# jizongFox/MI-based-Regularized-Semi-supervised-Segmentation

Measured on NVIDIA B200. Metric: iic_mi_loss_fwd_bwd_mpixels_per_s, higher is better.
Workload: dtype f32

## Files before the change

mi-based-regularized-semi-supervised-segmentation_b200/csrc/local_bwd_tcrb10h.cu:

```cuda
#include <cuda_fp16.h>
#include <stdlib.h>

#include "common.cuh"
#include "local_kernels.cuh"
#include "tc_common.cuh"
#include "tma.cuh"

namespace iic {
namespace bwdrb10h {
using namespace tc;

constexpr int T = 3, PAD = 1;
constexpr int KP = 16;
constexpr int RMAX = 8;
constexpr int TBUF = 2 * RMAX * KP;
constexpr int APX = 272;
constexpr int MAXW = 248;
constexpr int A_CHUNK = APX * 16;
constexpr int A_SLOT = 4 * A_CHUNK;
constexpr int NA = 6;
constexpr int RAW_SLOT = 10 * 256 * 4;
constexpr int NRAW = 6;
constexpr int WROWS = T * KP;
constexpr int W_TILE = 2 * WROWS * 16;
constexpr int W_IMG = 6 * W_TILE;
constexpr int NTHREADS = 704;
constexpr int NTHREADS_FL = 704;
constexpr int SMEM_BYTES = NA * A_SLOT + 2 * W_IMG + NRAW * RAW_SLOT + 1024;
constexpr int NL = 4;
constexpr int SMEM_BYTES_FL = SMEM_BYTES + NL * RAW_SLOT;
constexpr float A_SCALE = 256.f;
constexpr int A_SCALE_LOG2 = 8;
constexpr int W_TARGET_LOG2 = 12;



#ifdef IIC_TC_TRACE
__device__ long long g_trace[4][64][6];
__device__ long long g_ctrace[32][8];
#define TRACE(role, slot) do { if (blockIdx.x == 0 && tt >= 16 && tt < 80) g_trace[role][tt - 16][slot] = clock64(); } while (0)
#define CTRACE(slot) do { if (blockIdx.x == 0 && i < 32) g_ctrace[i][slot] = clock64(); } while (0)
#else
#define TRACE(role, slot) do { } while (0)
#define CTRACE(slot) do { } while (0)
#endif

struct Params {
  int B, H, W, K;
  const float* Wc[2];
  int Kp4;
  const float* grad_loss;
  float* out[2];
  long long out_sn[2];
  int from_logits;
  float inv_temp;
  const float* lout[2];
  long long l_sn[2], l_sc[2], l_sh[2];
};

__device__ __forceinline__ uint32_t pack_h2(float a, float b) {
  const __half2 p = __floats2half2_rn(a, b);
  return *reinterpret_cast<const uint32_t*>(&p);
}
__device__ __forceinline__ uint4 pack_h8(const float* v) {
  return make_uint4(pack_h2(v[0], v[1]), pack_h2(v[2], v[3]), pack_h2(v[4], v[5]), pack_h2(v[6], v[7]));
}
__device__ __forceinline__ void split_h(float v, float& h, float& l) {
  h = __half2float(__float2half_rn(v));
  l = __half2float(__float2half_rn(v - h));
}

__device__ __forceinline__ void build_weight_row(const float* __restrict__ Wc, unsigned char* img, int e, int K, int Kp4, float wscale) {
  const int row = e % WROWS, tx = e / WROWS;
  const int ty = T - 1 - row / KP, o = row % KP;
  float w1[10], w2[10];
#pragma unroll
  for (int c = 0; c < 10; ++c) {
    const float v = (c < K && o < K) ? __ldg(Wc + ((size_t)c * T * T + ty * T + tx) * Kp4 + o) * wscale : 0.f;
    split_h(v, w1[c], w2[c]);
  }
  const float c0[8] = {w1[0], w1[1], w1[2], w1[3], w1[4], w1[5], w1[6], w1[7]};
  const float c1[8] = {w1[8], w1[9], w1[0], w1[1], w1[2], w1[3], w1[4], w1[5]};
  const float c2[8] = {w1[6], w1[7], w1[8], w1[9], w2[0], w2[1], w2[2], w2[3]};
  const float c3[8] = {w2[4], w2[5], w2[6], w2[7], w2[8], w2[9], 0.f, 0.f};
  uint4* t = reinterpret_cast<uint4*>(img + (size_t)tx * 2 * W_TILE);
  t[row] = pack_h8(c0);
  t[WROWS + row] = pack_h8(c1);
  t[2 * WROWS + row] = pack_h8(c2);
  t[3 * WROWS + row] = pack_h8(c3);
}

struct Chunk { int n, h0, nr, q0; bool cont_next; };
__device__ __forceinline__ Chunk next_chunk(long long r, long long R0, long long R1, int H, int rc) {
  Chunk c;
  c.n = (int)(r / H);
  c.h0 = (int)(r - (long long)c.n * H);
  int run = H - c.h0;
  if (run > R1 - r) run = (int)(R1 - r);
  c.nr = rc < run ? rc : run;
  if (run - c.nr == 1 && c.nr >= 3) c.nr -= 1;
  c.q0 = (r > R0 && c.h0 > 0) ? 2 : 0;
  c.cont_next = c.nr < run;
  return c;
}

template <bool FROM_LOGITS>
__global__ void __launch_bounds__(FROM_LOGITS ? NTHREADS_FL : NTHREADS, 1)
local_bwd_tcrb10h_kernel(const __grid_constant__ CUtensorMap map0, const __grid_constant__ CUtensorMap map1, const Params P) {
  extern __shared__ __align__(1024) unsigned char smem_dyn[];
  __shared__ __align__(8) uint64_t raw_full[NRAW], raw_empty[NRAW], a_full[NA], a_empty[NA], w_full, accum_full[2], tmem_ready[2];
  __shared__ __align__(8) uint64_t l_full[NL], l_empty[NL];
  __shared__ uint32_t tmem_base_s;
  __shared__ float wmax_s[4];
  __shared__ float unscale_s;
  unsigned char* smem = smem_dyn + ((1024u - (smem_u32(smem_dyn) & 1023u)) & 1023u);
  unsigned char* a_ring = smem;
  unsigned char* w_img = smem + NA * A_SLOT;
  unsigned char* raw_ring = w_img + 2 * W_IMG;
  unsigned char* l_ring = raw_ring + NRAW * RAW_SLOT;
  const int wid = threadIdx.x >> 5, lane = threadIdx.x & 31;
  const long long rows_total = (long long)P.B * P.H;
  const long long R0 = (long long)blockIdx.x * rows_total / gridDim.x;
  const long long R1 = (long long)(blockIdx.x + 1) * rows_total / gridDim.x;
  const int share = (int)(R1 - R0);
  const int nch = (share + RMAX - 1) / RMAX;
  const int rc = nch > 0 ? (share + nch - 1) / nch : RMAX;
  const int SW = P.W + 8;
  const int raw_bytes = P.K * SW * 4;
  const int ntile = P.W > 128 ? 2 : 1;

  if (threadIdx.x == 0) {
    for (int s = 0; s < NRAW; ++s) { mbar_init(&raw_full[s], 1); mbar_init(&raw_empty[s], 4); }
    for (int s = 0; s < NA; ++s) { mbar_init(&a_full[s], 4); mbar_init(&a_empty[s], 2); }
    mbar_init(&w_full, 4);
    const int ndset_i = ntile == 2 ? 2 : 1;
    for (int s = 0; s < 2; ++s) { mbar_init(&accum_full[s], 4); mbar_init(&tmem_ready[s], 4 * ndset_i); }
    for (int s = 0; s < NL; ++s) { mbar_init(&l_full[s], 1); mbar_init(&l_empty[s], 4 * ndset_i); }
    mbar_fence_init();
  }
  if (wid == 3) {
    asm volatile("tcgen05.alloc.cta_group::1.sync.aligned.shared::cta.b32 [%0], %1;" ::"r"(smem_u32(&tmem_base_s)), "r"(512));
    asm volatile("tcgen05.relinquish_alloc_permit.cta_group::1.sync.aligned;");
  }
  asm volatile("tcgen05.fence::before_thread_sync;");
  __syncthreads();
  asm volatile("tcgen05.fence::after_thread_sync;");
  const uint32_t tmem_base = tmem_base_s;

  if (wid == 0) {
    if (lane == 0) {
      tma_prefetch_desc(&map0);
      tma_prefetch_desc(&map1);
      int t = 0, s = 0;
      unsigned sph = 0;
      for (int sweep = 0; sweep < 2; ++sweep)
      for (long long r = R0; r < R1;) {
        const Chunk c = next_chunk(r, R0, R1, P.H, rc);
        for (int q = c.q0; q < c.nr + T - 1; ++q, ++t) {
          { const int tt = t; (void)tt; TRACE(0, 0); }
          if (t >= NRAW) mbar_wait(&raw_empty[s], sph ^ 1u, 1);
          { const int tt = t; (void)tt; TRACE(0, 1); }
          mbar_arrive_expect_tx(&raw_full[s], raw_bytes);
          tma_load_4d(raw_ring + s * RAW_SLOT, sweep == 0 ? &map0 : &map1, &raw_full[s], -4, c.h0 - PAD + q, 0, c.n);
          if (++s == NRAW) { s = 0; sph ^= 1u; }
        }
        r += c.nr;
      }
    }
  } else if (wid == 3) {
    if (FROM_LOGITS && lane == 0) {
      int t = 0, s = 0;
      unsigned sph = 0;
      for (int sweep = 0; sweep < 2; ++sweep)
      for (long long r = R0; r < R1;) {
        const Chunk c = next_chunk(r, R0, R1, P.H, rc);
        for (int orow = 0; orow < c.nr; ++orow, ++t) {
          if (t >= NL) mbar_wait(&l_empty[s], sph ^ 1u, 9);
          mbar_arrive_expect_tx(&l_full[s], raw_bytes);
          tma_load_4d(l_ring + s * RAW_SLOT, sweep == 0 ? &map1 : &map0, &l_full[s], -4, c.h0 + orow, 0, c.n);
          if (++s == NL) { s = 0; sph ^= 1u; }
        }
        r += c.nr;
      }
    }
  } else if (wid == 1 || wid == 2 || wid == 12 || wid == 13) {
    const int mt = (wid == 1 || wid == 12) ? 0 : 1;
    const int par = wid >= 12 ? 1 : 0;
    const bool mine = mt < ntile;
    mbar_wait(&w_full, 0u, 7);
    const uint64_t w_base0 = make_desc_kmajor_noswz(smem_u32(w_img), WROWS * 16);
    static_assert(NA % 2 == 0 && NRAW % 2 == 0, "the stage-parity split needs even ring depths");
    int a = 0, i = 0, tt = 0;
    unsigned aph = 0;
    for (int sweep = 0; sweep < 2; ++sweep)
    for (long long r = R0; r < R1; ++i) {
      const uint64_t w_base = w_base0 + (uint64_t)(sweep * (W_IMG / 16));
      const Chunk c = next_chunk(r, R0, R1, P.H, rc);
      const int buf = i & 1;
      if (lane == 0 && wid == 1) CTRACE(0);
      mbar_wait(&tmem_ready[buf], (unsigned)(i >> 1) & 1u, 6);
      if (lane == 0 && wid == 1) CTRACE(1);
      asm volatile("tcgen05.fence::after_thread_sync;");
      const int nq = c.nr + T - 1;
      const int nr_next = c.cont_next ? next_chunk(r + c.nr, R0, R1, P.H, rc).nr : 0;
      for (int q = c.q0; q < nq; ++q, ++tt) {
        if ((tt & 1) != par) {
          if (++a == NA) { a = 0; aph ^= 1u; }
          continue;
        }
        if (lane == 0 && par == 0) TRACE(1 + mt, 0);
        mbar_wait(&a_full[a], aph, 5);
        asm volatile("tcgen05.fence::after_thread_sync;");
        if (lane == 0) {
          if (par == 0) TRACE(1 + mt, 1);
          if (mine) {
            const int ty_max = q < T - 1 ? q : T - 1;
            const int ty_min = q - c.nr + 1 > 0 ? q - c.nr + 1 : 0;
            const uint32_t nn = (uint32_t)((ty_max - ty_min + 1) * KP);
            const uint32_t idesc_f16 = (1u << 4) | ((nn >> 3) << 17) | (8u << 24);
            const uint32_t d_tmem = tmem_base + (uint32_t)(buf * TBUF + (mt * RMAX + (q - ty_max)) * KP);
            const uint64_t a_12 = make_desc_kmajor_noswz(smem_u32(a_ring + a * A_SLOT), A_CHUNK) + (uint64_t)(mt * 128 + 8 - PAD);
            const uint64_t a_34 = a_12 + (uint64_t)(2 * A_CHUNK / 16);
            const uint64_t b_base = w_base + (uint64_t)((T - 1 - ty_max) * KP);
#pragma unroll
            for (int tx = 0; tx < T; ++tx) {
              const uint64_t bt = b_base + (uint64_t)tx * (2 * W_TILE / 16);
              umma_bf16(d_tmem, a_12 + (uint64_t)tx, bt, idesc_f16);
              umma_bf16(d_tmem, a_34 + (uint64_t)tx, bt + (uint64_t)(W_TILE / 16), idesc_f16);
            }
          }
        }
        if (c.cont_next && q >= c.nr) {
          mbar_wait(&tmem_ready[buf ^ 1], (unsigned)((i + 1) >> 1) & 1u, 6);
          asm volatile("tcgen05.fence::after_thread_sync;");
          if (lane == 0 && mine) {
            const int q2 = q - c.nr;
            const int ty_max = q2;
            const int ty_min = q2 - nr_next + 1 > 0 ? q2 - nr_next + 1 : 0;
            const uint32_t nn = (uint32_t)((ty_max - ty_min + 1) * KP);
            const uint32_t idesc_f16 = (1u << 4) | ((nn >> 3) << 17) | (8u << 24);
            const uint32_t d_tmem = tmem_base + (uint32_t)((buf ^ 1) * TBUF + (mt * RMAX + (q2 - ty_max)) * KP);
            const uint64_t a_12 = make_desc_kmajor_noswz(smem_u32(a_ring + a * A_SLOT), A_CHUNK) + (uint64_t)(mt * 128 + 8 - PAD);
            const uint64_t a_34 = a_12 + (uint64_t)(2 * A_CHUNK / 16);
            const uint64_t b_base = w_base + (uint64_t)((T - 1 - ty_max) * KP);
#pragma unroll
            for (int tx = 0; tx < T; ++tx) {
              const uint64_t bt = b_base + (uint64_t)tx * (2 * W_TILE / 16);
              umma_bf16(d_tmem, a_12 + (uint64_t)tx, bt, idesc_f16);
              umma_bf16(d_tmem, a_34 + (uint64_t)tx, bt + (uint64_t)(W_TILE / 16), idesc_f16);
            }
          }
        }
        if (lane == 0) {
          if (par == 0) TRACE(1 + mt, 2);
          umma_commit(&a_empty[a]);
        }
        __syncwarp();
        if (++a == NA) { a = 0; aph ^= 1u; }
      }
      if (lane == 0) umma_commit(&accum_full[buf]);
      __syncwarp();
      r += c.nr;
    }
  } else if (wid >= 4 && wid < 12) {
    const int tid = (threadIdx.x - 128) & 127;
    const int grp = wid >= 8 ? 1 : 0;
    int a = 0, s = 0, t = 0;
    unsigned aph = 0, sph = 0;
    for (int sweep = 0; sweep < 2; ++sweep)
    for (long long r = R0; r < R1;) {
      const Chunk c = next_chunk(r, R0, R1, P.H, rc);
      for (int q = c.q0; q < c.nr + T - 1; ++q, ++t) {
        if ((t & 1) != grp) {
          if (++a == NA) { a = 0; aph ^= 1u; }
          if (++s == NRAW) { s = 0; sph ^= 1u; }
          continue;
        }
        const int tt = t;
        (void)tt;
        if (tid == 0 && wid == 4) TRACE(3, 0);
        if (t >= NA) mbar_wait(&a_empty[a], aph ^ 1u, 3);
        if (tid == 0 && wid == 4) TRACE(3, 1);
        mbar_wait(&raw_full[s], sph, 4);
        if (tid == 0 && wid == 4) TRACE(3, 2);
        unsigned char* am = a_ring + a * A_SLOT;
        const float* raw = reinterpret_cast<const float*>(raw_ring + s * RAW_SLOT);
        const int srow = c.h0 - PAD + q;
        const bool row_in = srow >= 0 && srow < P.H;
        float v[2][10];
#pragma unroll
        for (int u = 0; u < 2; ++u) {
          const int px = tid + u * 128;
#pragma unroll
          for (int ch = 0; ch < 10; ++ch) v[u][ch] = (ch < P.K && px < SW) ? raw[ch * SW + px] : 0.f;
        }
#pragma unroll
        for (int u = 0; u < 2; ++u) {
          const int px = tid + u * 128;
          if (FROM_LOGITS) {
            const int col = px - 4;
            if (row_in && col >= 0 && col < P.W) {
              float mx = v[u][0];
#pragma unroll
              for (int ch = 1; ch < 10; ++ch) if (ch < P.K) mx = fmaxf(mx, v[u][ch]);
              float sum = 0.f;
#pragma unroll
              for (int ch = 0; ch < 10; ++ch) {
                v[u][ch] = ch < P.K ? __expf((v[u][ch] - mx) * P.inv_temp) : 0.f;
                sum += v[u][ch];
              }
              const float inv = 1.f / sum;
#pragma unroll
              for (int ch = 0; ch < 10; ++ch) v[u][ch] *= inv;
            } else {
#pragma unroll
              for (int ch = 0; ch < 10; ++ch) v[u][ch] = 0.f;
            }
          }
        }
        float2 hi[10], lo[10];
#pragma unroll
        for (int ch = 0; ch < 10; ++ch) {
          const float2 sv = __fmul2_rn(make_float2(v[0][ch], v[1][ch]), make_float2(A_SCALE, A_SCALE));
          hi[ch] = make_float2(__uint_as_float(__float_as_uint(sv.x) & 0xFFFFE000u), __uint_as_float(__float_as_uint(sv.y) & 0xFFFFE000u));
          lo[ch] = __ffma2_rn(hi[ch], make_float2(-1.f, -1.f), sv);
        }
#pragma unroll
        for (int u = 0; u < 2; ++u) {
          const int px = tid + u * 128;
          uint32_t hp[5], lp[5];
#pragma unroll
          for (int c2 = 0; c2 < 5; ++c2) {
            const __half2 hh = u == 0 ? __floats2half2_rn(hi[2 * c2].x, hi[2 * c2 + 1].x) : __floats2half2_rn(hi[2 * c2].y, hi[2 * c2 + 1].y);
            const __half2 ll = u == 0 ? __floats2half2_rn(lo[2 * c2].x, lo[2 * c2 + 1].x) : __floats2half2_rn(lo[2 * c2].y, lo[2 * c2 + 1].y);
            hp[c2] = *reinterpret_cast<const uint32_t*>(&hh);
            lp[c2] = *reinterpret_cast<const uint32_t*>(&ll);
          }
          if (px < SW) {
            const int off = (px + 4) * 16;
            *reinterpret_cast<uint4*>(am + off) = make_uint4(hp[0], hp[1], hp[2], hp[3]);
            *reinterpret_cast<uint4*>(am + A_CHUNK + off) = make_uint4(hp[4], lp[0], lp[1], lp[2]);
            *reinterpret_cast<uint4*>(am + 2 * A_CHUNK + off) = make_uint4(lp[3], lp[4], hp[0], hp[1]);
            *reinterpret_cast<uint4*>(am + 3 * A_CHUNK + off) = make_uint4(hp[2], hp[3], hp[4], 0u);
          }
        }
        __syncwarp();
        if (lane == 0) mbar_arrive(&raw_empty[s]);
        asm volatile("fence.proxy.async.shared::cta;" ::: "memory");
        __syncwarp();
        if (lane == 0) mbar_arrive(&a_full[a]);
        if (tid == 0 && wid == 4) TRACE(3, 3);
        if (++a == NA) { a = 0; aph ^= 1u; }
        if (++s == NRAW) { s = 0; sph ^= 1u; }
      }
      r += c.nr;
    }
  } else if (wid >= 14) {
    const int q4 = wid & 3;
    const int dset = wid >= 18 ? 1 : 0;
    const int ndset = ntile == 2 ? 2 : 1;
    const int mt0 = ndset == 2 ? dset : 0, mt1 = ndset == 2 ? dset + 1 : ntile;
    const int zc0 = ndset == 2 ? dset * RMAX * KP : 0, zc1 = ndset == 2 ? (dset + 1) * RMAX * KP : TBUF;
    float unscale = 1.f;
    const float g0 = P.grad_loss ? __ldg(P.grad_loss) : 1.f;
    const size_t plane = (size_t)P.H * P.W;
    const uint32_t lane_base = tmem_base + ((uint32_t)(q4 * 32) << 16);
    auto zero_accumulators = [&](int buf) {
      for (int c = zc0; c < zc1; c += 8)
        asm volatile("tcgen05.st.sync.aligned.32x32b.x8.b32 [%0], {%1, %1, %1, %1, %1, %1, %1, %1};" ::"r"(lane_base + buf * TBUF + c), "r"(0u) : "memory");
      asm volatile("tcgen05.wait::st.sync.aligned;" ::: "memory");
      asm volatile("tcgen05.fence::before_thread_sync;");
      __syncwarp();
      if (lane == 0) mbar_arrive(&tmem_ready[buf]);
    };
    if (dset < ndset) {
    zero_accumulators(0);
    zero_accumulators(1);
    }
    if (dset == 0) {
      const int etid = threadIdx.x - 14 * 32;
      const int ncoef = P.K * T * T * P.Kp4;
      float mx = 0.f;
      for (int e = etid; e < 2 * ncoef; e += 128) mx = fmaxf(mx, fabsf(__ldg(P.Wc[e >= ncoef] + (e >= ncoef ? e - ncoef : e))));
#pragma unroll
      for (int o = 16; o > 0; o >>= 1) mx = fmaxf(mx, __shfl_xor_sync(0xffffffffu, mx, o));
      if (lane == 0) wmax_s[q4] = mx;
      asm volatile("bar.sync 1, 128;" ::: "memory");
      mx = fmaxf(fmaxf(wmax_s[0], wmax_s[1]), fmaxf(wmax_s[2], wmax_s[3]));
      int wexp = 0;
      if (mx > 0.f && mx < 3.0e38f) wexp = W_TARGET_LOG2 - ilogbf(mx);
      if (wexp > 100) wexp = 100;
      const float wscale = scalbnf(1.f, wexp);
      unscale = scalbnf(1.f, -(wexp + A_SCALE_LOG2));
      for (int e = etid; e < 2 * 3 * WROWS; e += 128) {
        const int sweep = e / (3 * WROWS);
        build_weight_row(P.Wc[sweep], w_img + sweep * W_IMG, e - sweep * 3 * WROWS, P.K, P.Kp4, wscale);
      }
      if (etid == 0) unscale_s = unscale;
      asm volatile("fence.proxy.async.shared::cta;" ::: "memory");
      __syncwarp();
      if (lane == 0) mbar_arrive(&w_full);
    } else {
      mbar_wait(&w_full, 0u, 7);
      unscale = *reinterpret_cast<volatile float*>(&unscale_s);
    }
    const float g = g0 * unscale;
    int i = 0, ls = 0;
    unsigned lph = 0;
    for (int sweep = 0; sweep < 2 && dset < ndset; ++sweep)
    for (long long r = R0; r < R1; ++i) {
      const Chunk c = next_chunk(r, R0, R1, P.H, rc);
      const int buf = i & 1;
      if (lane == 0 && wid == 14) CTRACE(2);
      mbar_wait(&accum_full[buf], (unsigned)(i >> 1) & 1u, 8);
      if (lane == 0 && wid == 14) CTRACE(3);
      asm volatile("tcgen05.fence::after_thread_sync;");
      for (int orow = 0; orow < c.nr; orow += 2) {
        const int nrow = orow + 1 < c.nr ? 2 : 1;
        if (FROM_LOGITS) {
          mbar_wait(&l_full[ls], lph, 10);
          if (nrow == 2) mbar_wait(&l_full[(ls + 1) % NL], (ls + 1 == NL) ? (lph ^ 1u) : lph, 10);
        }
        for (int mt = mt0; mt < mt1; ++mt) {
          const int col = mt * 128 + q4 * 32 + lane;
          const bool live = col < P.W;
          uint32_t v[2][16];
#pragma unroll
          for (int h = 0; h < 2; ++h) {
            const int orh = orow + h < RMAX ? orow + h : orow;
#pragma unroll
            for (int ch = 0; ch < 16; ch += 8) {
              const uint32_t taddr = lane_base + (uint32_t)(buf * TBUF + (mt * RMAX + orh) * KP + ch);
              asm volatile("tcgen05.ld.sync.aligned.32x32b.x8.b32 {%0, %1, %2, %3, %4, %5, %6, %7}, [%8];"
                           : "=r"(v[h][ch]), "=r"(v[h][ch + 1]), "=r"(v[h][ch + 2]), "=r"(v[h][ch + 3]), "=r"(v[h][ch + 4]),
                             "=r"(v[h][ch + 5]), "=r"(v[h][ch + 6]), "=r"(v[h][ch + 7])
                           : "r"(taddr));
            }
          }
          asm volatile("tcgen05.wait::ld.sync.aligned;" ::: "memory");
          if (live) {
#pragma unroll
            for (int h = 0; h < 2; ++h) {
              if (h < nrow) {
                float* dst = P.out[sweep] + (size_t)c.n * P.out_sn[sweep] + (size_t)(c.h0 + orow + h) * P.W + col;
                if (!FROM_LOGITS) {
                  if (P.K == 10) {
#pragma unroll
                    for (int o = 0; o < 10; ++o) dst[(size_t)o * plane] = g * __uint_as_float(v[h][o]);
                  } else {
#pragma unroll
                    for (int o = 0; o < 9; ++o) dst[(size_t)o * plane] = g * __uint_as_float(v[h][o]);
                  }
                } else {
                  const float* lp = reinterpret_cast<const float*>(l_ring + ((ls + h) % NL) * RAW_SLOT) + col + 4;
                  float pr[10];
                  float mx = -3.0e38f;
#pragma unroll
                  for (int o = 0; o < 10; ++o) {
                    pr[o] = o < P.K ? lp[o * SW] : -3.0e38f;
                    mx = fmaxf(mx, pr[o]);
                  }
                  float sum = 0.f;
#pragma unroll
                  for (int o = 0; o < 10; ++o) {
                    pr[o] = o < P.K ? __expf((pr[o] - mx) * P.inv_temp) : 0.f;
                    sum += pr[o];
                  }
                  const float inv = 1.f / sum;
                  float dot = 0.f;
#pragma unroll
                  for (int o = 0; o < 10; ++o) {
                    pr[o] *= inv;
                    dot = fmaf(g * __uint_as_float(v[h][o]), pr[o], dot);
                  }
                  if (P.K == 10) {
#pragma unroll
                    for (int o = 0; o < 10; ++o) dst[(size_t)o * plane] = P.inv_temp * pr[o] * (g * __uint_as_float(v[h][o]) - dot);
                  } else {
#pragma unroll
                    for (int o = 0; o < 9; ++o) dst[(size_t)o * plane] = P.inv_temp * pr[o] * (g * __uint_as_float(v[h][o]) - dot);
                  }
                }
              }
            }
          }
        }
        if (FROM_LOGITS) {
          __syncwarp();
          for (int h = 0; h < nrow; ++h) {
            if (lane == 0) mbar_arrive(&l_empty[ls]);
            if (++ls == NL) { ls = 0; lph ^= 1u; }
          }
        }
      }
      r += c.nr;
      if (lane == 0 && wid == 14) CTRACE(4);
      zero_accumulators(buf);
      if (lane == 0 && wid == 14) CTRACE(5);
    }
  }
  asm volatile("tcgen05.fence::before_thread_sync;");
  __syncthreads();
  if (wid == 3) asm volatile("tcgen05.dealloc.cta_group::1.sync.aligned.b32 %0, %1;" ::"r"(tmem_base), "r"(512));
}

}

int local_bwd_tcrb10h_try(const LocalMaps& m, const float* Wx, const float* Wy, const LocalGrads& g, int from_logits,
                          float inv_temp, cudaStream_t st) {
  using namespace bwdrb10h;
  const int B = m.B, K = m.K, H = m.H, W = m.W, sms = m.sms;
  if ((K != 9 && K != 10) || m.pad != 1 || W % 4 != 0 || W > MAXW || W < 8) return -1;
  if ((long long)B * H < 8LL * sms && !options().tc10_force) return -1;
  CUtensorMap mx, my;
  if (!make_map_4d(&mx, m.x, m, W + 8, 1, K)) return -1;
  if (!make_map_4d(&my, m.y, m, W + 8, 1, K)) return -1;
  IIC_CHECK_RC(ensure_dyn_smem((const void*)(local_bwd_tcrb10h_kernel<false>), (int)(SMEM_BYTES)));
  IIC_CHECK_RC(ensure_dyn_smem((const void*)(local_bwd_tcrb10h_kernel<true>), (int)(SMEM_BYTES_FL)));
  const int Kp4 = (K + 3) & ~3;
  Params P{B, H, W, K, {Wx, Wy}, Kp4, g.grad_loss, {g.gx, g.gy}, {g.gx_sn, g.gy_sn}, from_logits, inv_temp, {m.x.p, m.y.p},
           {m.x.sn, m.y.sn}, {m.x.sc, m.y.sc}, {m.x.sh, m.y.sh}};
  if (from_logits) local_bwd_tcrb10h_kernel<true><<<sms, NTHREADS_FL, SMEM_BYTES_FL, st>>>(my, mx, P);
  else local_bwd_tcrb10h_kernel<false><<<sms, NTHREADS, SMEM_BYTES, st>>>(my, mx, P);
  IIC_CHECK_CUDA(cudaGetLastError());
  return 0;
}

}
```

Before: 9992.

## Fold horizontal taps into MMA N dimension and combine via warp shuffles

The backward local conv no longer issues three separate UMMA pairs per row, one per horizontal tap tx. It widens N to 32 so that all three tx taps for the 10 outputs come out of one MMA. The epilogue then shifts the tx=0 and tx=2 partial sums by one column with warp shuffles, using a small shared-memory exchange at warp boundaries, and adds them to the centre tap. Tiles overlap, at 126 columns per tile, to supply halo columns. RMAX is halved, the parity-split second MMA warp pair is removed, and chunk-boundary MMAs are deferred with held ring slots. The aim is fewer MMA issues and less weight footprint, at the cost of extra TMEM loads, shuffles and a named barrier in the epilogue.

```diff
diff --git a/mi-based-regularized-semi-supervised-segmentation_b200/csrc/local_bwd_tcrb10h.cu b/mi-based-regularized-semi-supervised-segmentation_b200/csrc/local_bwd_tcrb10h.cu
--- a/mi-based-regularized-semi-supervised-segmentation_b200/csrc/local_bwd_tcrb10h.cu
+++ b/mi-based-regularized-semi-supervised-segmentation_b200/csrc/local_bwd_tcrb10h.cu
@@ -11,9 +11,10 @@
 using namespace tc;
 
 constexpr int T = 3, PAD = 1;
-constexpr int KP = 16;
-constexpr int RMAX = 8;
-constexpr int TBUF = 2 * RMAX * KP;
+constexpr int TW = 126;
+constexpr int NO = 32;
+constexpr int RMAX = 4;
+constexpr int TBUF = 2 * RMAX * NO;
 constexpr int APX = 272;
 constexpr int MAXW = 248;
 constexpr int A_CHUNK = APX * 16;
@@ -21,11 +22,11 @@
 constexpr int NA = 6;
 constexpr int RAW_SLOT = 10 * 256 * 4;
 constexpr int NRAW = 6;
-constexpr int WROWS = T * KP;
+constexpr int WROWS = T * NO;
 constexpr int W_TILE = 2 * WROWS * 16;
-constexpr int W_IMG = 6 * W_TILE;
-constexpr int NTHREADS = 704;
-constexpr int NTHREADS_FL = 704;
+constexpr int W_IMG = 2 * W_TILE;
+constexpr int NTHREADS = 640;
+constexpr int NTHREADS_FL = 640;
 constexpr int SMEM_BYTES = NA * A_SLOT + 2 * W_IMG + NRAW * RAW_SLOT + 1024;
 constexpr int NL = 4;
 constexpr int SMEM_BYTES_FL = SMEM_BYTES + NL * RAW_SLOT;
@@ -65,25 +66,33 @@
 __device__ __forceinline__ uint4 pack_h8(const float* v) {
   return make_uint4(pack_h2(v[0], v[1]), pack_h2(v[2], v[3]), pack_h2(v[4], v[5]), pack_h2(v[6], v[7]));
 }
+__device__ __forceinline__ void tmem_ld10(uint32_t taddr, float (&v)[10]) {
+  uint32_t u[10];
+#pragma unroll
+  for (int k = 0; k < 10; k += 2)
+    asm volatile("tcgen05.ld.sync.aligned.32x32b.x2.b32 {%0, %1}, [%2];" : "=r"(u[k]), "=r"(u[k + 1]) : "r"(taddr + (uint32_t)k));
+#pragma unroll
+  for (int k = 0; k < 10; ++k) v[k] = __uint_as_float(u[k]);
+}
 __device__ __forceinline__ void split_h(float v, float& h, float& l) {
   h = __half2float(__float2half_rn(v));
   l = __half2float(__float2half_rn(v - h));
 }
 
-__device__ __forceinline__ void build_weight_row(const float* __restrict__ Wc, unsigned char* img, int e, int K, int Kp4, float wscale) {
-  const int row = e % WROWS, tx = e / WROWS;
-  const int ty = T - 1 - row / KP, o = row % KP;
+__device__ __forceinline__ void build_weight_row(const float* __restrict__ Wc, unsigned char* img, int row, int K, int Kp4, float wscale) {
+  const int ty = T - 1 - row / NO, j = row % NO;
+  const int tx = j / 10, o = j % 10;
   float w1[10], w2[10];
 #pragma unroll
   for (int c = 0; c < 10; ++c) {
-    const float v = (c < K && o < K) ? __ldg(Wc + ((size_t)c * T * T + ty * T + tx) * Kp4 + o) * wscale : 0.f;
+    const float v = (c < K && o < K && tx < T) ? __ldg(Wc + ((size_t)c * T * T + ty * T + tx) * Kp4 + o) * wscale : 0.f;
     split_h(v, w1[c], w2[c]);
   }
   const float c0[8] = {w1[0], w1[1], w1[2], w1[3], w1[4], w1[5], w1[6], w1[7]};
   const float c1[8] = {w1[8], w1[9], w1[0], w1[1], w1[2], w1[3], w1[4], w1[5]};
   const float c2[8] = {w1[6], w1[7], w1[8], w1[9], w2[0], w2[1], w2[2], w2[3]};
   const float c3[8] = {w2[4], w2[5], w2[6], w2[7], w2[8], w2[9], 0.f, 0.f};
-  uint4* t = reinterpret_cast<uint4*>(img + (size_t)tx * 2 * W_TILE);
+  uint4* t = reinterpret_cast<uint4*>(img);
   t[row] = pack_h8(c0);
   t[WROWS + row] = pack_h8(c1);
   t[2 * WROWS + row] = pack_h8(c2);
@@ -113,6 +122,7 @@
   __shared__ uint32_t tmem_base_s;
   __shared__ float wmax_s[4];
   __shared__ float unscale_s;
+  __shared__ __align__(16) float xchg_s[2][2][RMAX * 4 * 24];
   unsigned char* smem = smem_dyn + ((1024u - (smem_u32(smem_dyn) & 1023u)) & 1023u);
   unsigned char* a_ring = smem;
   unsigned char* w_img = smem + NA * A_SLOT;
@@ -127,14 +137,14 @@
   const int rc = nch > 0 ? (share + nch - 1) / nch : RMAX;
   const int SW = P.W + 8;
   const int raw_bytes = P.K * SW * 4;
-  const int ntile = P.W > 128 ? 2 : 1;
+  const int ntile = P.W > TW ? 2 : 1;
 
   if (threadIdx.x == 0) {
     for (int s = 0; s < NRAW; ++s) { mbar_init(&raw_full[s], 1); mbar_init(&raw_empty[s], 4); }
     for (int s = 0; s < NA; ++s) { mbar_init(&a_full[s], 4); mbar_init(&a_empty[s], 2); }
     mbar_init(&w_full, 4);
     const int ndset_i = ntile == 2 ? 2 : 1;
-    for (int s = 0; s < 2; ++s) { mbar_init(&accum_full[s], 4); mbar_init(&tmem_ready[s], 4 * ndset_i); }
+    for (int s = 0; s < 2; ++s) { mbar_init(&accum_full[s], 2); mbar_init(&tmem_ready[s], 4 * ndset_i); }
     for (int s = 0; s < NL; ++s) { mbar_init(&l_full[s], 1); mbar_init(&l_empty[s], 4 * ndset_i); }
     mbar_fence_init();
   }
@@ -183,15 +193,25 @@
         r += c.nr;
       }
     }
-  } else if (wid == 1 || wid == 2 || wid == 12 || wid == 13) {
-    const int mt = (wid == 1 || wid == 12) ? 0 : 1;
-    const int par = wid >= 12 ? 1 : 0;
+  } else if (wid == 1 || wid == 2) {
+    const int mt = wid - 1;
     const bool mine = mt < ntile;
     mbar_wait(&w_full, 0u, 7);
     const uint64_t w_base0 = make_desc_kmajor_noswz(smem_u32(w_img), WROWS * 16);
-    static_assert(NA % 2 == 0 && NRAW % 2 == 0, "the stage-parity split needs even ring depths");
+    static_assert(NA % 2 == 0 && NRAW % 2 == 0, "the transform groups' stage-parity split needs even ring depths");
     int a = 0, i = 0, tt = 0;
     unsigned aph = 0;
+    int held0 = 0, held1 = 0;
+    auto issue = [&](int slot, int bufc, int orow0, int ty_min, int ty_max, uint64_t w_base) {
+      const uint32_t nn = (uint32_t)((ty_max - ty_min + 1) * NO);
+      const uint32_t idesc_f16 = (1u << 4) | ((nn >> 3) << 17) | (8u << 24);
+      const uint32_t d_tmem = tmem_base + (uint32_t)(bufc * TBUF + (mt * RMAX + orow0) * NO);
+      const uint64_t a_12 = make_desc_kmajor_noswz(smem_u32(a_ring + slot * A_SLOT), A_CHUNK) + (uint64_t)(mt * TW + 8 - PAD);
+      const uint64_t a_34 = a_12 + (uint64_t)(2 * A_CHUNK / 16);
+      const uint64_t bt = w_base + (uint64_t)((T - 1 - ty_max) * NO);
+      umma_bf16(d_tmem, a_12, bt, idesc_f16);
+      umma_bf16(d_tmem, a_34, bt + (uint64_t)(W_TILE / 16), idesc_f16);
+    };
     for (int sweep = 0; sweep < 2; ++sweep)
     for (long long r = R0; r < R1; ++i) {
       const uint64_t w_base = w_base0 + (uint64_t)(sweep * (W_IMG / 16));
@@ -201,59 +221,34 @@
       mbar_wait(&tmem_ready[buf], (unsigned)(i >> 1) & 1u, 6);
       if (lane == 0 && wid == 1) CTRACE(1);
       asm volatile("tcgen05.fence::after_thread_sync;");
+      if (c.q0 == 2) {
+        if (lane == 0) {
+          if (mine) {
+            issue(held0, buf, 0, 0, 0, w_base);
+            issue(held1, buf, 0, 2 - c.nr > 0 ? 2 - c.nr : 0, 1, w_base);
+          }
+          umma_commit(&a_empty[held0]);
+          umma_commit(&a_empty[held1]);
+        }
+        __syncwarp();
+      }
       const int nq = c.nr + T - 1;
-      const int nr_next = c.cont_next ? next_chunk(r + c.nr, R0, R1, P.H, rc).nr : 0;
       for (int q = c.q0; q < nq; ++q, ++tt) {
-        if ((tt & 1) != par) {
-          if (++a == NA) { a = 0; aph ^= 1u; }
-          continue;
-        }
-        if (lane == 0 && par == 0) TRACE(1 + mt, 0);
+        if (lane == 0) TRACE(1 + mt, 0);
         mbar_wait(&a_full[a], aph, 5);
         asm volatile("tcgen05.fence::after_thread_sync;");
         if (lane == 0) {
-          if (par == 0) TRACE(1 + mt, 1);
-          if (mine) {
-            const int ty_max = q < T - 1 ? q : T - 1;
-            const int ty_min = q - c.nr + 1 > 0 ? q - c.nr + 1 : 0;
-            const uint32_t nn = (uint32_t)((ty_max - ty_min + 1) * KP);
-            const uint32_t idesc_f16 = (1u << 4) | ((nn >> 3) << 17) | (8u << 24);
-            const uint32_t d_tmem = tmem_base + (uint32_t)(buf * TBUF + (mt * RMAX + (q - ty_max)) * KP);
-            const uint64_t a_12 = make_desc_kmajor_noswz(smem_u32(a_ring + a * A_SLOT), A_CHUNK) + (uint64_t)(mt * 128 + 8 - PAD);
-            const uint64_t a_34 = a_12 + (uint64_t)(2 * A_CHUNK / 16);
-            const uint64_t b_base = w_base + (uint64_t)((T - 1 - ty_max) * KP);
-#pragma unroll
-            for (int tx = 0; tx < T; ++tx) {
-              const uint64_t bt = b_base + (uint64_t)tx * (2 * W_TILE / 16);
-              umma_bf16(d_tmem, a_12 + (uint64_t)tx, bt, idesc_f16);
-              umma_bf16(d_tmem, a_34 + (uint64_t)tx, bt + (uint64_t)(W_TILE / 16), idesc_f16);
-            }
-          }
-        }
-        if (c.cont_next && q >= c.nr) {
-          mbar_wait(&tmem_ready[buf ^ 1], (unsigned)((i + 1) >> 1) & 1u, 6);
-          asm volatile("tcgen05.fence::after_thread_sync;");
-          if (lane == 0 && mine) {
-            const int q2 = q - c.nr;
-            const int ty_max = q2;
-            const int ty_min = q2 - nr_next + 1 > 0 ? q2 - nr_next + 1 : 0;
-            const uint32_t nn = (uint32_t)((ty_max - ty_min + 1) * KP);
-            const uint32_t idesc_f16 = (1u << 4) | ((nn >> 3) << 17) | (8u << 24);
-            const uint32_t d_tmem = tmem_base + (uint32_t)((buf ^ 1) * TBUF + (mt * RMAX + (q2 - ty_max)) * KP);
-            const uint64_t a_12 = make_desc_kmajor_noswz(smem_u32(a_ring + a * A_SLOT), A_CHUNK) + (uint64_t)(mt * 128 + 8 - PAD);
-            const uint64_t a_34 = a_12 + (uint64_t)(2 * A_CHUNK / 16);
-            const uint64_t b_base = w_base + (uint64_t)((T - 1 - ty_max) * KP);
-#pragma unroll
-            for (int tx = 0; tx < T; ++tx) {
-              const uint64_t bt = b_base + (uint64_t)tx * (2 * W_TILE / 16);
-              umma_bf16(d_tmem, a_12 + (uint64_t)tx, bt, idesc_f16);
-              umma_bf16(d_tmem, a_34 + (uint64_t)tx, bt + (uint64_t)(W_TILE / 16), idesc_f16);
-            }
-          }
-        }
-        if (lane == 0) {
-          if (par == 0) TRACE(1 + mt, 2);
-          umma_commit(&a_empty[a]);
+          TRACE(1 + mt, 1);
+          const int ty_max = q < T - 1 ? q : T - 1;
+          const int ty_min = q - c.nr + 1 > 0 ? q - c.nr + 1 : 0;
+          if (mine) issue(a, buf, q - ty_max, ty_min, ty_max, w_base);
+          TRACE(1 + mt, 2);
+          if (c.cont_next && q >= c.nr) {
+            if (q == c.nr) held0 = a;
+            else held1 = a;
+          } else {
+            umma_commit(&a_empty[a]);
+          }
         }
         __syncwarp();
         if (++a == NA) { a = 0; aph ^= 1u; }
@@ -355,12 +350,12 @@
       }
       r += c.nr;
     }
-  } else if (wid >= 14) {
+  } else if (wid >= 12) {
     const int q4 = wid & 3;
-    const int dset = wid >= 18 ? 1 : 0;
+    const int dset = wid >= 16 ? 1 : 0;
     const int ndset = ntile == 2 ? 2 : 1;
     const int mt0 = ndset == 2 ? dset : 0, mt1 = ndset == 2 ? dset + 1 : ntile;
-    const int zc0 = ndset == 2 ? dset * RMAX * KP : 0, zc1 = ndset == 2 ? (dset + 1) * RMAX * KP : TBUF;
+    const int zc0 = ndset == 2 ? dset * RMAX * NO : 0, zc1 = ndset == 2 ? (dset + 1) * RMAX * NO : TBUF;
     float unscale = 1.f;
     const float g0 = P.grad_loss ? __ldg(P.grad_loss) : 1.f;
     const size_t plane = (size_t)P.H * P.W;
@@ -378,7 +373,7 @@
     zero_accumulators(1);
     }
     if (dset == 0) {
-      const int etid = threadIdx.x - 14 * 32;
+      const int etid = threadIdx.x - 12 * 32;
       const int ncoef = P.K * T * T * P.Kp4;
       float mx = 0.f;
       for (int e = etid; e < 2 * ncoef; e += 128) mx = fmaxf(mx, fabsf(__ldg(P.Wc[e >= ncoef] + (e >= ncoef ? e - ncoef : e))));
@@ -392,9 +387,9 @@
       if (wexp > 100) wexp = 100;
       const float wscale = scalbnf(1.f, wexp);
       unscale = scalbnf(1.f, -(wexp + A_SCALE_LOG2));
-      for (int e = etid; e < 2 * 3 * WROWS; e += 128) {
-        const int sweep = e / (3 * WROWS);
-        build_weight_row(P.Wc[sweep], w_img + sweep * W_IMG, e - sweep * 3 * WROWS, P.K, P.Kp4, wscale);
+      for (int e = etid; e < 2 * WROWS; e += 128) {
+        const int sweep = e / WROWS;
+        build_weight_row(P.Wc[sweep], w_img + sweep * W_IMG, e - sweep * WROWS, P.K, P.Kp4, wscale);
       }
       if (etid == 0) unscale_s = unscale;
       asm volatile("fence.proxy.async.shared::cta;" ::: "memory");
@@ -405,16 +400,45 @@
       unscale = *reinterpret_cast<volatile float*>(&unscale_s);
     }
     const float g = g0 * unscale;
-    int i = 0, ls = 0;
+    int i = 0, ls = 0, xpar = 0;
     unsigned lph = 0;
     for (int sweep = 0; sweep < 2 && dset < ndset; ++sweep)
     for (long long r = R0; r < R1; ++i) {
       const Chunk c = next_chunk(r, R0, R1, P.H, rc);
       const int buf = i & 1;
-      if (lane == 0 && wid == 14) CTRACE(2);
+      if (lane == 0 && wid == 12) CTRACE(2);
       mbar_wait(&accum_full[buf], (unsigned)(i >> 1) & 1u, 8);
-      if (lane == 0 && wid == 14) CTRACE(3);
+      if (lane == 0 && wid == 12) CTRACE(3);
       asm volatile("tcgen05.fence::after_thread_sync;");
+      float* xs = &xchg_s[dset][xpar][0];
+      for (int orow = 0; orow < c.nr; ++orow) {
+        const uint32_t taddr = lane_base + (uint32_t)(buf * TBUF + (mt0 * RMAX + orow) * NO);
+        uint32_t u[NO];
+            asm volatile("tcgen05.ld.sync.aligned.32x32b.x16.b32 {%0, %1, %2, %3, %4, %5, %6, %7, %8, %9, %10, %11, %12, %13, %14, %15}, [%16];"
+                         : "=r"(u[0]), "=r"(u[1]), "=r"(u[2]), "=r"(u[3]), "=r"(u[4]), "=r"(u[5]), "=r"(u[6]), "=r"(u[7]),
+                           "=r"(u[8]), "=r"(u[9]), "=r"(u[10]), "=r"(u[11]), "=r"(u[12]), "=r"(u[13]), "=r"(u[14]), "=r"(u[15])
+                         : "r"(taddr));
+            asm volatile("tcgen05.ld.sync.aligned.32x32b.x16.b32 {%0, %1, %2, %3, %4, %5, %6, %7, %8, %9, %10, %11, %12, %13, %14, %15}, [%16];"
+                         : "=r"(u[16]), "=r"(u[17]), "=r"(u[18]), "=r"(u[19]), "=r"(u[20]), "=r"(u[21]), "=r"(u[22]), "=r"(u[23]),
+                           "=r"(u[24]), "=r"(u[25]), "=r"(u[26]), "=r"(u[27]), "=r"(u[28]), "=r"(u[29]), "=r"(u[30]), "=r"(u[31])
+                         : "r"(taddr + 16u));
+            asm volatile("tcgen05.wait::ld.sync.aligned;" ::: "memory");
+        if (lane == 31) {
+          float4* d = reinterpret_cast<float4*>(xs + (orow * 4 + q4) * 24);
+          d[0] = make_float4(__uint_as_float(u[0]), __uint_as_float(u[1]), __uint_as_float(u[2]), __uint_as_float(u[3]));
+          d[1] = make_float4(__uint_as_float(u[4]), __uint_as_float(u[5]), __uint_as_float(u[6]), __uint_as_float(u[7]));
+          d[2] = make_float4(__uint_as_float(u[8]), __uint_as_float(u[9]), 0.f, 0.f);
+        }
+        if (lane == 0) {
+          float4* d = reinterpret_cast<float4*>(xs + (orow * 4 + q4) * 24 + 12);
+          d[0] = make_float4(__uint_as_float(u[20]), __uint_as_float(u[21]), __uint_as_float(u[22]), __uint_as_float(u[23]));
+          d[1] = make_float4(__uint_as_float(u[24]), __uint_as_float(u[25]), __uint_as_float(u[26]), __uint_as_float(u[27]));
+          d[2] = make_float4(__uint_as_float(u[28]), __uint_as_float(u[29]), 0.f, 0.f);
+        }
+      }
+      if (dset == 0) asm volatile("bar.sync 2, 128;" ::: "memory");
+      else asm volatile("bar.sync 3, 128;" ::: "memory");
+      xpar ^= 1;
       for (int orow = 0; orow < c.nr; orow += 2) {
         const int nrow = orow + 1 < c.nr ? 2 : 1;
         if (FROM_LOGITS) {
@@ -422,64 +446,79 @@
           if (nrow == 2) mbar_wait(&l_full[(ls + 1) % NL], (ls + 1 == NL) ? (lph ^ 1u) : lph, 10);
         }
         for (int mt = mt0; mt < mt1; ++mt) {
-          const int col = mt * 128 + q4 * 32 + lane;
-          const bool live = col < P.W;
-          uint32_t v[2][16];
-#pragma unroll
-          for (int h = 0; h < 2; ++h) {
-            const int orh = orow + h < RMAX ? orow + h : orow;
-#pragma unroll
-            for (int ch = 0; ch < 16; ch += 8) {
-              const uint32_t taddr = lane_base + (uint32_t)(buf * TBUF + (mt * RMAX + orh) * KP + ch);
-              asm volatile("tcgen05.ld.sync.aligned.32x32b.x8.b32 {%0, %1, %2, %3, %4, %5, %6, %7}, [%8];"
-                           : "=r"(v[h][ch]), "=r"(v[h][ch + 1]), "=r"(v[h][ch + 2]), "=r"(v[h][ch + 3]), "=r"(v[h][ch + 4]),
-                             "=r"(v[h][ch + 5]), "=r"(v[h][ch + 6]), "=r"(v[h][ch + 7])
-                           : "r"(taddr));
+          const int m = q4 * 32 + lane;
+          const int col = mt * TW + m - 1;
+          const bool live = m >= 1 && m <= TW && col < P.W;
+          for (int h = 0; h < nrow; ++h) {
+            const uint32_t taddr = lane_base + (uint32_t)(buf * TBUF + (mt * RMAX + orow + h) * NO);
+            uint32_t u[NO];
+            asm volatile("tcgen05.ld.sync.aligned.32x32b.x16.b32 {%0, %1, %2, %3, %4, %5, %6, %7, %8, %9, %10, %11, %12, %13, %14, %15}, [%16];"
+                         : "=r"(u[0]), "=r"(u[1]), "=r"(u[2]), "=r"(u[3]), "=r"(u[4]), "=r"(u[5]), "=r"(u[6]), "=r"(u[7]),
+                           "=r"(u[8]), "=r"(u[9]), "=r"(u[10]), "=r"(u[11]), "=r"(u[12]), "=r"(u[13]), "=r"(u[14]), "=r"(u[15])
+                         : "r"(taddr));
+            asm volatile("tcgen05.ld.sync.aligned.32x32b.x16.b32 {%0, %1, %2, %3, %4, %5, %6, %7, %8, %9, %10, %11, %12, %13, %14, %15}, [%16];"
+                         : "=r"(u[16]), "=r"(u[17]), "=r"(u[18]), "=r"(u[19]), "=r"(u[20]), "=r"(u[21]), "=r"(u[22]), "=r"(u[23]),
+                           "=r"(u[24]), "=r"(u[25]), "=r"(u[26]), "=r"(u[27]), "=r"(u[28]), "=r"(u[29]), "=r"(u[30]), "=r"(u[31])
+                         : "r"(taddr + 16u));
+            asm volatile("tcgen05.wait::ld.sync.aligned;" ::: "memory");
+            float d0[10], d2[10], s[10];
+#pragma unroll
+            for (int o = 0; o < 10; ++o) {
+              d0[o] = __shfl_up_sync(0xffffffffu, __uint_as_float(u[o]), 1);
+              d2[o] = __shfl_down_sync(0xffffffffu, __uint_as_float(u[20 + o]), 1);
             }
-          }
-          asm volatile("tcgen05.wait::ld.sync.aligned;" ::: "memory");
-          if (live) {
-#pragma unroll
-            for (int h = 0; h < 2; ++h) {
-              if (h < nrow) {
-                float* dst = P.out[sweep] + (size_t)c.n * P.out_sn[sweep] + (size_t)(c.h0 + orow + h) * P.W + col;
-                if (!FROM_LOGITS) {
-                  if (P.K == 10) {
-#pragma unroll
-                    for (int o = 0; o < 10; ++o) dst[(size_t)o * plane] = g * __uint_as_float(v[h][o]);
-                  } else {
-#pragma unroll
-                    for (int o = 0; o < 9; ++o) dst[(size_t)o * plane] = g * __uint_as_float(v[h][o]);
-                  }
+            if (lane == 0 && q4 > 0) {
+              const float4* e = reinterpret_cast<const float4*>(xs + ((orow + h) * 4 + q4 - 1) * 24);
+              const float4 a = e[0], b = e[1], c2 = e[2];
+              d0[0] = a.x; d0[1] = a.y; d0[2] = a.z; d0[3] = a.w; d0[4] = b.x; d0[5] = b.y; d0[6] = b.z; d0[7] = b.w;
+              d0[8] = c2.x; d0[9] = c2.y;
+            }
+            if (lane == 31 && q4 < 3) {
+              const float4* e = reinterpret_cast<const float4*>(xs + ((orow + h) * 4 + q4 + 1) * 24 + 12);
+              const float4 a = e[0], b = e[1], c2 = e[2];
+              d2[0] = a.x; d2[1] = a.y; d2[2] = a.z; d2[3] = a.w; d2[4] = b.x; d2[5] = b.y; d2[6] = b.z; d2[7] = b.w;
+              d2[8] = c2.x; d2[9] = c2.y;
+            }
+#pragma unroll
+            for (int o = 0; o < 10; ++o) s[o] = (d0[o] + d2[o]) + __uint_as_float(u[10 + o]);
+            if (live) {
+              float* dst = P.out[sweep] + (size_t)c.n * P.out_sn[sweep] + (size_t)(c.h0 + orow + h) * P.W + col;
+              if (!FROM_LOGITS) {
+                if (P.K == 10) {
+#pragma unroll
+                  for (int o = 0; o < 10; ++o) dst[(size_t)o * plane] = g * s[o];
                 } else {
-                  const float* lp = reinterpret_cast<const float*>(l_ring + ((ls + h) % NL) * RAW_SLOT) + col + 4;
-                  float pr[10];
-                  float mx = -3.0e38f;
-#pragma unroll
-                  for (int o = 0; o < 10; ++o) {
-                    pr[o] = o < P.K ? lp[o * SW] : -3.0e38f;
-                    mx = fmaxf(mx, pr[o]);
-                  }
-                  float sum = 0.f;
-#pragma unroll
-                  for (int o = 0; o < 10; ++o) {
-                    pr[o] = o < P.K ? __expf((pr[o] - mx) * P.inv_temp) : 0.f;
-                    sum += pr[o];
-                  }
-                  const float inv = 1.f / sum;
-                  float dot = 0.f;
-#pragma unroll
-                  for (int o = 0; o < 10; ++o) {
-                    pr[o] *= inv;
-                    dot = fmaf(g * __uint_as_float(v[h][o]), pr[o], dot);
-                  }
-                  if (P.K == 10) {
-#pragma unroll
-                    for (int o = 0; o < 10; ++o) dst[(size_t)o * plane] = P.inv_temp * pr[o] * (g * __uint_as_float(v[h][o]) - dot);
-                  } else {
-#pragma unroll
-                    for (int o = 0; o < 9; ++o) dst[(size_t)o * plane] = P.inv_temp * pr[o] * (g * __uint_as_float(v[h][o]) - dot);
-                  }
+#pragma unroll
+                  for (int o = 0; o < 9; ++o) dst[(size_t)o * plane] = g * s[o];
+                }
+              } else {
+                const float* lp = reinterpret_cast<const float*>(l_ring + ((ls + h) % NL) * RAW_SLOT) + col + 4;
+                float pr[10];
+                float mx = -3.0e38f;
+#pragma unroll
+                for (int o = 0; o < 10; ++o) {
+                  pr[o] = o < P.K ? lp[o * SW] : -3.0e38f;
+                  mx = fmaxf(mx, pr[o]);
+                }
+                float sum = 0.f;
+#pragma unroll
+                for (int o = 0; o < 10; ++o) {
+                  pr[o] = o < P.K ? __expf((pr[o] - mx) * P.inv_temp) : 0.f;
+                  sum += pr[o];
+                }
+                const float inv = 1.f / sum;
+                float dot = 0.f;
+#pragma unroll
+                for (int o = 0; o < 10; ++o) {
+                  pr[o] *= inv;
+                  dot = fmaf(g * s[o], pr[o], dot);
+                }
+                if (P.K == 10) {
+#pragma unroll
+                  for (int o = 0; o < 10; ++o) dst[(size_t)o * plane] = P.inv_temp * pr[o] * (g * s[o] - dot);
+                } else {
+#pragma unroll
+                  for (int o = 0; o < 9; ++o) dst[(size_t)o * plane] = P.inv_temp * pr[o] * (g * s[o] - dot);
                 }
               }
             }
@@ -494,9 +533,9 @@
         }
       }
       r += c.nr;
-      if (lane == 0 && wid == 14) CTRACE(4);
+      if (lane == 0 && wid == 12) CTRACE(4);
       zero_accumulators(buf);
-      if (lane == 0 && wid == 14) CTRACE(5);
+      if (lane == 0 && wid == 12) CTRACE(5);
     }
   }
   asm volatile("tcgen05.fence::before_thread_sync;");
```

Result: slower. 8883 (median of 6 runs) (-11.1%).
